# 1chizhang/OpenDCVC

Hardware: AMD Instinct MI355X
Metric: 1080p YUV420 encode+decode FPS (frames/s through encode AND decode, whole job) (higher is better)
Workload: dtype f16

## Files before the change

### opendcvc_amd/csrc/dcb_t128.hpp

```cpp
#pragma once

namespace t128 {

typedef float floatx16 __attribute__((ext_vector_type(16)));

constexpr int TW = 16, TH = 8, M = TW * TH;
constexpr int NW = 8, NTHR = NW * 64;
constexpr int PT = M / 32;
constexpr int PTW = PT / 2;
constexpr int PAD = 8;
constexpr int VC = 64, LDV = VC + PAD;
constexpr int HALO = (TH + 2) * (TW + 2);
constexpr int DW_SLAB = 64;
constexpr int LDS_S = DW_SLAB;

constexpr int PADF = 24;

struct G128 {
    static constexpr int TW = t128::TW, TH = t128::TH, NW = t128::NW, D = 8, DW_SLAB = t128::DW_SLAB, WPS = 2;
};
struct G32 {
    static constexpr int TW = 8, TH = 4, NW = 4, D = 24 , DW_SLAB = 128, WPS = 1;
};
template <class G>
struct Geo : G {
    static constexpr int M = G::TW * G::TH, NTHR = G::NW * 64;
    static constexpr int PTW = (M / 32) / (G::NW / 4);
    static constexpr int HALO = (G::TH + 2) * (G::TW + 2);
    static constexpr int LDS_S = G::DW_SLAB;
    static_assert(M % 32 == 0 && PTW >= 1 && G::NW % 4 == 0, "tile geometry");
};

template <int C>
struct Wcfg {
    static_assert(C % 64 == 0, "DepthConvBlock widths are padded to 64");
    static constexpr int NT = C / 32;
    static constexpr int NTW = (NT + 3) / 4;
    static constexpr bool RAG = NT % 4 != 0;
    static constexpr int KS = C / 16;
    static constexpr int NCH = 2 * C / VC;
    static constexpr int F4 = 4 * NTW;
    static constexpr int LDX = C + PAD;
    static constexpr int FRAGS = KS * NTW + NCH * KS + NCH * F4;
    static constexpr int STREAM = FRAGS + PADF;
};

template <int C, class G = G128, bool HEADIN = false>
struct Cfg : Wcfg<C> {
    using GE = Geo<G>;
    using WC = Wcfg<C>;
    using WC::NT; using WC::NTW; using WC::RAG; using WC::KS; using WC::NCH; using WC::F4; using WC::LDX; using WC::FRAGS; using WC::STREAM;
    static_assert(C % G::DW_SLAB == 0, "whole depthwise slabs");
    static constexpr int D = G::D;
    static_assert(D <= PADF, "stream padding");
    static constexpr size_t slab_elems = (size_t)(HEADIN && C / G::DW_SLAB > 2 ? C / G::DW_SLAB : 2) * GE::HALO * GE::LDS_S;
    static constexpr size_t v_elems = (size_t)2 * GE::M * LDV > slab_elems ? (size_t)2 * GE::M * LDV : slab_elems;
    static constexpr size_t TAB_BYTES = (size_t)9 * C * 2 + (size_t)C * 4 + (size_t)4 * C * 4;
    static constexpr int HROWS = (GE::HALO + 31) / 32 * 32;
    static constexpr size_t HEAD_BYTES = HEADIN ? (size_t)HROWS * LDX * sizeof(half_t) : 0;
    static constexpr size_t LDS = ((size_t)GE::M * LDX + v_elems) * sizeof(half_t) + TAB_BYTES + HEAD_BYTES;
    static_assert(LDS <= 160 * 1024, "LDS budget");
    static_assert(NCH % 2 == 0 && NCH >= 4, "the chunk loop is unrolled by two");
    static_assert((2 * C) % VC == 0, "whole FFN chunks");
    static constexpr int OFF_U0 = (KS * NTW) % D;
    static constexpr int OFF_S0 = (OFF_U0 + KS) % D;
    static constexpr int OFF_ODD = (OFF_S0 + KS) % D;
    static constexpr int OFF_EVEN = (OFF_ODD + F4 + KS) % D;
    static_assert((2 * (F4 + KS)) % D == 0, "the two-step loop body must turn the ring a whole number of times");
    static constexpr int OFF_LAST = OFF_ODD;
    static constexpr int OFF_FIN = (OFF_LAST + F4) % D;
};

__device__ __forceinline__ floatx16 mfma32(const half8& a, const half8& b, const floatx16& c)
{
    return __builtin_amdgcn_mfma_f32_32x32x16_f16(a, b, c, 0, 0, 0);
}


template <int C, class G = G128, bool HEADIN = false>
__global__ __launch_bounds__(Geo<G>::NTHR, G::WPS) void dcb_tail128_kernel(TailParams p)
{
    using TR = Traits<half_t>;
    using CF = Cfg<C, G, HEADIN>;
    using GE = Geo<G>;
    constexpr int TW = GE::TW, TH = GE::TH, M = GE::M, NTHR = GE::NTHR, PTW = GE::PTW, HALO = GE::HALO, DW_SLAB = GE::DW_SLAB,
                  LDS_S = GE::LDS_S;
    constexpr int NTW = CF::NTW, KS = CF::KS, NCH = CF::NCH, D = CF::D, LDX = CF::LDX, V = 8, GC = C / V;
    extern __shared__ __attribute__((aligned(32))) char smem[];
    half_t* bufX = reinterpret_cast<half_t*>(smem);
    half_t* bufV = bufX + M * LDX;
    half_t* tabW = bufV + CF::v_elems;
    float* tabBd = reinterpret_cast<float*>(tabW + 9 * C);
    float* tabB3 = tabBd + C;
    const int tid = threadIdx.x, lane = tid & 63;
    const int wave = __builtin_amdgcn_readfirstlane(tid >> 6);
    const int cqw = wave & 3, ph = wave >> 2;
    const int pl = lane & 31, hh = lane >> 5;
    const int tiles_x = (p.W + TW - 1) / TW;
    const int ty0 = (blockIdx.x / tiles_x) * TH, tx0 = (blockIdx.x % tiles_x) * TW;
    const half_t* a = reinterpret_cast<const half_t*>(p.a);
    const half_t* ident = reinterpret_cast<const half_t*>(p.ident);
    [[maybe_unused]] unsigned long long ts0 = 0, ts1 = 0, ts2 = 0, ts3 = 0, ts4 = 0, ts5 = 0, ts6 = 0;
    [[maybe_unused]] unsigned long long td[8] = {0, 0, 0, 0, 0, 0, 0, 0};
    STAMP(ts0);

    const __amdgpu_buffer_rsrc_t wrsrc = __builtin_amdgcn_make_buffer_rsrc(
        const_cast<char*>(reinterpret_cast<const char*>(p.wt)) + (size_t)cqw * CF::STREAM * 1024, 0, CF::STREAM * 1024, 0x00020000);
    const int wlane = lane * 16;
    int woff = 0;
    auto wload = [&]() __attribute__((always_inline)) {
        typedef unsigned u32x4 __attribute__((ext_vector_type(4)));
        const u32x4 v = __builtin_amdgcn_raw_buffer_load_b128(wrsrc, wlane, woff, 0);
        woff += 1024;
        return __builtin_bit_cast(half8, v);
    };
    half8 ring[D];

    constexpr int HW_ = TW + 2, GS = DW_SLAB / V, NLD = (HALO * GS + NTHR - 1) / NTHR;
    constexpr int nslab = C / DW_SLAB;
// ... 99 lines not shown
        }
#pragma unroll
        for (int i = 0; i < NTW; ++i) {
            const int chb = 32 * (cqw + 4 * i) + 4 * hh;
#pragma unroll
            for (int g = 0; g < 4; ++g) {
                const floatx4 bias = load_f4(p.hb1 + chb + 8 * g);
#pragma unroll
                for (int t = 0; t < HT; ++t) {
                    const int hp = 32 * t + pl;
                    const int y = ty0 - 1 + hp / HW_, x = tx0 - 1 + hp % HW_;
                    const bool inside = hp < HALO && y >= 0 && y < p.H && x >= 0 && x < p.W;
                    floatx4 v = {hacc[i][t][4 * g], hacc[i][t][4 * g + 1], hacc[i][t][4 * g + 2], hacc[i][t][4 * g + 3]};
                    v = v + bias;
#pragma unroll
                    for (int r = 0; r < 4; ++r) v[r] = inside ? TR::gate(v[r]) : 0.f;
                    const int ch = chb + 8 * g;
                    if (hp < HALO) lds_store_quad<half_t>(bufV + (ch / DW_SLAB) * (HALO * LDS_S), LDS_S, hp, ch % DW_SLAB, v);
                }
            }
        }
    }
    constexpr int NID = M * GC / NTHR;
    constexpr int G8 = C / 64, RPP = NTHR / 8;
    static_assert(M % RPP == 0 && NID == (M / RPP) * G8, "identity pass mapping");
    auto idmap = [&](int k, int& m, int& c) __attribute__((always_inline)) {
        c = ((tid & 7) + 8 * (k % G8)) * V;
        m = (tid >> 3) + RPP * (k / G8);
    };
    Vec16 idv[NID];
    const __amdgpu_buffer_rsrc_t irsrc = __builtin_amdgcn_make_buffer_rsrc(
        const_cast<half_t*>(ident), 0, (int)((long)p.H * p.W * p.ldi * 2), 0x00020000);
    auto ident_fetch = [&]() __attribute__((always_inline)) {
#pragma unroll
        for (int k = 0; k < NID; ++k) {
            int m, icg;
            idmap(k, m, icg);
            const int y = ty0 + m / TW, x = tx0 + m % TW;
            int off = (y < p.H && x < p.W) ? ((y * p.W + x) * (int)p.ldi + icg) * 2 : OOB;
#ifdef DCVC_DIAG
            if (p.ablate & 32) off = (tid & 255) * 16;
#endif
            idv[k] = __builtin_bit_cast(Vec16, __builtin_amdgcn_raw_buffer_load_b128(irsrc, off, 0, 0));
        }
    };

    const int prow = (ph * PTW) * 32 + pl;
    const half_t* xb = bufX + prow * LDX + 8 * hh;
    auto bfrag_x = [&](int t, int s) __attribute__((always_inline)) {
        return *reinterpret_cast<const half8*>(xb + t * 32 * LDX + s * 16);
    };

    floatx16 acc[NTW][PTW];
    half8 g2b[PTW];
    auto gemm2_slot = [&](int s, int q) __attribute__((always_inline)) {
        const int i = q / PTW, t = q % PTW, k = (s * NTW + i) % D;
        if (q == 0) {
#pragma unroll
            for (int tt = 0; tt < PTW; ++tt) g2b[tt] = bfrag_x(tt, s);
        }
        if (s == 0) {
            floatx16 zero;
#pragma unroll
            for (int r = 0; r < 16; ++r) zero[r] = 0.f;
            acc[i][t] = mfma32(ring[k], g2b[t], zero);
        } else {
            acc[i][t] = mfma32(ring[k], g2b[t], acc[i][t]);
        }
        if (t == PTW - 1) ring[k] = wload();
    };
    constexpr int G2Q = NTW * PTW;
    {
        static_assert(NTHR / GS == M / 2 && TH % 2 == 0, "one pixel pair per thread and slab");
        const int pp = tid / GS, py = 2 * (pp / TW), px = pp % TW;
#pragma unroll
        for (int slab = 0; slab < nslab; ++slab) {
            half_t* hb = bufV + (HEADIN ? slab : (slab & 1)) * (HALO * LDS_S);
            if constexpr (!HEADIN) {
#pragma unroll
                for (int k = 0; k < NLD; ++k) {
                    const int hp = tid / GS + k * (NTHR / GS);
                    if (hp < HALO) *reinterpret_cast<Vec16*>(hb + hp * LDS_S + dcs) = pre[slab][k];
                }
            }
            if (slab == (nslab >= 2 ? nslab - 2 : 0)) ident_fetch();
            if (slab == nslab - 1) {
#pragma unroll
                for (int k = 0; k < D; ++k) ring[k] = wload();
            }
            if (slab == 0) STAMP(td[0]);
            __syncthreads();
            if (slab < 4) STAMP(td[1 + slab]);
            taps_fetch(slab);
            const int c = slab * DW_SLAB + dcs;
            Vec16 tv[4][3];
#pragma unroll
            for (int r = 0; r < 4; ++r)
#pragma unroll
                for (int kx = 0; kx < 3; ++kx)
                    tv[r][kx] = *reinterpret_cast<const Vec16*>(hb + ((py + r) * HW_ + px + kx) * LDS_S + dcs);
            __builtin_amdgcn_sched_barrier(0);
#pragma unroll
            for (int e = 0; e < 2; ++e) {
                float sacc[V];
#pragma unroll
                for (int j = 0; j < V; ++j) sacc[j] = 0.f;
#pragma unroll
                for (int ky = 0; ky < 3; ++ky)
#pragma unroll
                    for (int kx = 0; kx < 3; ++kx) fma_vec16<half_t>(tv[e + ky][kx], wtap[ky * 3 + kx], sacc);
#pragma unroll
                for (int j = 0; j < 4; ++j) {
                    sacc[j] = sacc[j] + bd0[j];
                    sacc[4 + j] = sacc[4 + j] + bd1[j];
                }
                lds_store_vec<half_t>(bufX, LDX, (py + e) * TW + px, c, pack16<half_t>(sacc));
            }
        }
        __syncthreads();
    }
    STAMP(ts1);

    auto tile_of = [&](int i) __attribute__((always_inline)) { return cqw + 4 * i; };
    auto tile_exists = [&](int i) __attribute__((always_inline)) { return !CF::RAG || cqw + 4 * i < CF::NT; };
    constexpr bool EB_PRE = NTW <= 2;
    floatx4 ebias[EB_PRE ? NTW : 1][4];
    auto ebias_load = [&](const float* b) __attribute__((always_inline)) {
        if constexpr (EB_PRE) {
#pragma unroll
            for (int i = 0; i < NTW; ++i)
#pragma unroll
                for (int g = 0; g < 4; ++g) ebias[i][g] = load_f4(b + 32 * tile_of(i) + 4 * hh + 8 * g);
        }
    };
    auto ebias_get = [&](const float* b, int i, int g) __attribute__((always_inline)) {
        if constexpr (EB_PRE) return ebias[i][g];
        return load_f4(b + 32 * tile_of(i) + 4 * hh + 8 * g);
    };
    ebias_load(p.b2);

#pragma unroll
    for (int mm = 0; mm < KS * G2Q; ++mm) {
        gemm2_slot(mm / G2Q, mm % G2Q);
        __builtin_amdgcn_sched_barrier(0);
    }
    auto gemm_c = [&](auto next) __attribute__((always_inline)) {
        half8 bc[PTW], bn[PTW];
#pragma unroll
        for (int t = 0; t < PTW; ++t) bc[t] = bfrag_x(t, 0);
        floatx16 zero;
#pragma unroll
        for (int r = 0; r < 16; ++r) zero[r] = 0.f;
        __builtin_amdgcn_sched_barrier(0);
#pragma unroll
        for (int s = 0; s < KS; ++s) {
// ... 27 lines not shown
    }
    __syncthreads();
#pragma unroll
    for (int k = 0; k < NID; ++k) {
        int m, icg;
        idmap(k, m, icg);
        const half8 o = __builtin_bit_cast(half8, lds_load_vec<half_t>(bufX, LDX, m, icg)) + __builtin_bit_cast(half8, idv[k]);
        lds_store_vec<half_t>(bufX, LDX, m, icg, __builtin_bit_cast(Vec16, o));
    }
    __syncthreads();

    STAMP(ts3);
#pragma unroll
    for (int i = 0; i < NTW; ++i)
#pragma unroll
        for (int t = 0; t < PTW; ++t)
#pragma unroll
            for (int r = 0; r < 16; ++r) acc[i][t][r] = 0.f;
    floatx16 ua[PTW], ub[PTW];
    const float* b3w = tabB3 + 16 * cqw + 4 * hh;
    floatx16 biasv;
    auto bias_load = [&](int j) __attribute__((always_inline)) {
        j = j < NCH ? j : NCH - 1;
        const floatx4 l0 = load_f4(b3w + 64 * j), l1 = load_f4(b3w + 64 * j + 8);
        const floatx4 h0 = load_f4(b3w + 64 * j + 2 * C), h1 = load_f4(b3w + 64 * j + 2 * C + 8);
#pragma unroll
        for (int r = 0; r < 4; ++r) {
            biasv[r] = l0[r];
            biasv[4 + r] = l1[r];
            biasv[8 + r] = h0[r];
            biasv[12 + r] = h1[r];
        }
    };
    constexpr int NPIECE = 4 * PTW * 6;
    float ge[4], gr[4];
    floatx4 vq;
    auto gate_piece = [&](const floatx16 (&u)[PTW], half_t* vbuf, int i) __attribute__((always_inline)) {
        const int n = i / 6, phs = i % 6, t = n >> 2, g = (n >> 1) & 1, hf = n & 1;
        const float lo0 = u[t][4 * g + 2 * hf], lo1 = u[t][4 * g + 2 * hf + 1];
        const float hi0 = u[t][8 + 4 * g + 2 * hf], hi1 = u[t][8 + 4 * g + 2 * hf + 1];
        if (phs == 0) {
            ge[0] = __builtin_amdgcn_exp2f(lo0);
            ge[1] = __builtin_amdgcn_exp2f(lo1);
        } else if (phs == 1) {
            ge[2] = __builtin_amdgcn_exp2f(hi0);
            ge[3] = __builtin_amdgcn_exp2f(hi1);
        } else if (phs == 2) {
            gr[0] = __builtin_amdgcn_rcpf(1.0f + ge[0]);
// ... 1 lines not shown
        } else if (phs == 3) {
            gr[2] = __builtin_amdgcn_rcpf(1.0f + ge[2]);
            gr[3] = __builtin_amdgcn_rcpf(1.0f + ge[3]);
        } else if (phs == 4) {
            vq[2 * hf] = DCVC_FMAF(hi0, gr[2], lo0 * gr[0]);
        } else {
            vq[2 * hf + 1] = DCVC_FMAF(hi1, gr[3], lo1 * gr[1]);
            if (hf == 1) lds_store_quad<half_t>(vbuf, LDV, prow + 32 * t, 16 * cqw + 8 * g + 4 * hh, vq);
        }
    };
    auto wload_ffn = [&]() __attribute__((always_inline)) {
#ifdef DCVC_DIAG
        if (p.ablate & 256) {
            typedef unsigned u32x4 __attribute__((ext_vector_type(4)));
            return __builtin_bit_cast(half8, __builtin_amdgcn_raw_buffer_load_b128(wrsrc, wlane, 0, 0));
        }
#endif
        return wload();
    };
    auto step = [&](auto G4c, auto G3c, auto GATEc, auto OFFc, const floatx16 (&ug)[PTW], floatx16 (&un)[PTW], half_t* vcur,
                    const half_t* vprev, int jb) __attribute__((always_inline)) {
        constexpr bool G4 = decltype(G4c)::value, G3 = decltype(G3c)::value, GATE = decltype(GATEc)::value;
        constexpr int OFF = decltype(OFFc)::value;
        constexpr int N4 = G4 ? 4 : 0, NS = N4 + (G3 ? KS : 0);
        constexpr int TM = N4 * NTW * PTW + (G3 ? KS * PTW : 0);
        constexpr int PPS = GATE ? (NPIECE + TM - 1) / TM : 0;
        auto load_b1 = [&](int idx, int t) __attribute__((always_inline)) {
#ifdef DCVC_DIAG
            if (p.ablate & 512) idx = idx < N4 ? 0 : N4;
#endif
            if (idx < N4) return *reinterpret_cast<const half8*>(vprev + (prow + 32 * t) * LDV + 8 * hh + idx * 16);
            return bfrag_x(t, idx - N4);
        };
        half8 bc[PTW], bn[PTW];
#pragma unroll
        for (int t = 0; t < PTW; ++t) bc[t] = load_b1(0, t);
        __builtin_amdgcn_sched_barrier(0);
        int m = 0;
#pragma unroll
        for (int idx = 0; idx < NS; ++idx) {
            const int nm = idx < N4 ? NTW * PTW : PTW;
#pragma unroll
            for (int q = 0; q < NTW * PTW; ++q) {
                if (q < nm) {
                    if (idx + 1 < NS && q < PTW) bn[q] = load_b1(idx + 1, q);
                    const int t = q % PTW;
                    if (idx < N4) {
// ... 638 lines not shown
```

### opendcvc_amd/csrc/dcvc_nn.hip

```cpp
#include <algorithm>
#include <cstdio>
#include <cstdlib>
#include <functional>
#include <memory>
#include <mutex>
#include <type_traits>
#include <unordered_map>
#include <vector>

#include "common.hpp"
#include "gemm_core.hpp"

namespace {

using dcvc::round_up;

template <int MT>
struct Tile {
    static constexpr int M = 16 * MT;
    static constexpr int TW = MT >= 8 ? 16 : 8;
    static constexpr int TH = M / TW;
};

#ifndef DCVC_PF_SMALL
// ... 841 lines not shown
{
    std::vector<float> v(n);
    for (int i = 0; i < n; ++i) v[i] = get(i);
    return dst.upload(v.data(), v.size() * sizeof(float));
}

template <typename T>
int upload_T(DevBuf& dst, int n, const std::function<float(int)>& get)
{
    std::vector<T> v(n);
    for (int i = 0; i < n; ++i) v[i] = (T)get(i);
    return dst.upload(v.data(), v.size() * sizeof(T));
}


}

struct dcvc_dcb {
    int dtype, cin, c, cin_p, c_p, shortcut, adapt;
    DevBuf wa, ba, w1, b1, wd, bd, w2, b2, w3, b3, w4, b4;
    DevBuf wa_t128;
    DevBuf w1_t128;
    DevBuf wt128;
};

struct dcvc_conv {
    int dtype, cin, cout, cin_p, n_p, cs_p, kh, kw, stride, pad, epi;
    DevBuf w, b;
    DevBuf w_t128;
    DevBuf w_c128[2];
    DevBuf w_s2;
};

namespace {

template <typename T, int MT>
size_t head_lds(int kstage, int c, bool adapt)
{
    const int kx = kstage > c ? kstage : c;
    return (size_t)Tile<MT>::M * ((kx + Traits<T>::kPad) + (adapt ? c + Traits<T>::kPad : 0)) * sizeof(T);
}
template <typename T, int MT, int NTW, int NW>
size_t tail_lds(int c)
{
    return TailLds<T, MT, TailCfg<MT, NTW, NW>::NTV, NW>::bytes(c);
}

template <typename T, int MT, int NTW, int NW, bool RAG = false, bool HEADIN = false>
int launch_tail(const TailParams& tp, int grid, int C, hipStream_t st)
{
    const size_t lds = TailLds<T, MT, TailCfg<MT, NTW, NW>::NTV, NW>::bytes(C, HEADIN);
    int rc = set_lds(dcb_tail_kernel<T, MT, NTW, NW, RAG, HEADIN>, lds);
// ... 4 lines not shown

template <typename K>
int set_lds(K kernel, size_t bytes)
{
    if (bytes > 160 * 1024) {
        dcvc::set_error("kernel needs %zu bytes of LDS (> 160 KiB)", bytes);
        return dcvc::E_ARG;
    }
    if (bytes > 64 * 1024) {
        static std::mutex mu;
        static std::unordered_map<const void*, size_t> granted;
        const void* key = reinterpret_cast<const void*>(kernel);
        std::lock_guard<std::mutex> lk(mu);
        size_t& have = granted[key];
        if (have < bytes) {
            DCVC_HIP(hipFuncSetAttribute(key, hipFuncAttributeMaxDynamicSharedMemorySize, (int)bytes));
            have = bytes;
        }
    }
    return 0;
}


template <int C>
int pack_t128(DevBuf& dst, const std::function<float(int, int)>& W2, const std::function<float(int, int)>& W3,
              const std::function<float(int, int)>& W4)
{
    using CF = t128::Wcfg<C>;
    std::vector<half_t> buf((size_t)4 * CF::STREAM * 512, (half_t)0.f);
    for (int wave = 0; wave < 4; ++wave) {
        size_t f = 0;
        auto put = [&](const std::function<float(int, int)>& get, const std::function<int(int)>& row, int s) {
            half_t* o = &buf[((size_t)wave * CF::STREAM + f) * 512];
            for (int l = 0; l < 64; ++l)
                for (int j = 0; j < 8; ++j) o[l * 8 + j] = (half_t)get(row(l & 31), 16 * s + 8 * (l >> 5) + j);
            ++f;
        };
        auto g3 = [&](int j) {
            for (int s = 0; s < CF::KS; ++s)
                put(W3, [&](int r) { return (r < 16 ? 0 : 2 * C - 16) + 64 * j + 16 * wave + r; }, s);
        };
        auto g4 = [&](int j) {
            for (int s4 = 0; s4 < 4; ++s4)
                for (int i = 0; i < CF::NTW; ++i) put(W4, [&](int r) { return 32 * (wave + 4 * i) + r; }, 4 * j + s4);
        };
        for (int s = 0; s < CF::KS; ++s)
            for (int i = 0; i < CF::NTW; ++i) put(W2, [&](int r) { return 32 * (wave + 4 * i) + r; }, s);
        g3(0);
        for (int j = 0; j < CF::NCH; ++j) {
            if (j >= 1) g4(j - 1);
            if (j + 1 < CF::NCH) g3(j + 1);
        }
        g4(CF::NCH - 1);
        if (f != (size_t)CF::FRAGS) {
            dcvc::set_error("pack_t128: %zu fragments packed, %d expected", f, CF::FRAGS);
            return dcvc::E_ARG;
        }
    }
    return dst.upload(buf.data(), buf.size() * sizeof(half_t));
}

inline bool t128_width_ok(int c_p) { return c_p == 128 || c_p == 256 || c_p == 320 || c_p == 384 || c_p == 512; }

template <int C>
int pack_t128_square(DevBuf& dst, const std::function<float(int, int)>& W)
{
    using CF = t128::Wcfg<C>;
    constexpr int LEN = CF::KS * CF::NTW + t128::PADF;
    std::vector<half_t> buf((size_t)4 * LEN * 512, (half_t)0.f);
    for (int cq = 0; cq < 4; ++cq) {
        size_t f = 0;
        for (int s = 0; s < CF::KS; ++s)
            for (int i = 0; i < CF::NTW; ++i, ++f) {
                half_t* o = &buf[((size_t)cq * LEN + f) * 512];
                for (int l = 0; l < 64; ++l)
                    for (int j = 0; j < 8; ++j) o[l * 8 + j] = (half_t)W(32 * (cq + 4 * i) + (l & 31), 16 * s + 8 * (l >> 5) + j);
            }
    }
    return dst.upload(buf.data(), buf.size() * sizeof(half_t));
}

template <int C>
int pack_t128_rect(DevBuf& dst, int Kp, const std::function<float(int, int)>& W)
{
    using CF = t128::Wcfg<C>;
    const int ks = Kp / 16, LEN = ks * CF::NTW + t128::PADF;
    std::vector<half_t> buf((size_t)4 * LEN * 512, (half_t)0.f);
    for (int cq = 0; cq < 4; ++cq) {
        size_t f = 0;
        for (int s = 0; s < ks; ++s)
            for (int i = 0; i < CF::NTW; ++i, ++f) {
                half_t* o = &buf[((size_t)cq * LEN + f) * 512];
                for (int l = 0; l < 64; ++l)
                    for (int j = 0; j < 8; ++j) o[l * 8 + j] = (half_t)W(32 * (cq + 4 * i) + (l & 31), 16 * s + 8 * (l >> 5) + j);
            }
    }
    return dst.upload(buf.data(), buf.size() * sizeof(half_t));
}

// ... 15 lines not shown
                    }
        }
    return dst.upload(buf.data(), buf.size() * sizeof(half_t));
}

template <typename F>
int visit_t128_width(int c_p, F&& f)
{
    switch (c_p) {
    case 128: return f(std::integral_constant<int, 128>());
    case 256: return f(std::integral_constant<int, 256>());
    case 320: return f(std::integral_constant<int, 320>());
    case 384: return f(std::integral_constant<int, 384>());
    case 512: return f(std::integral_constant<int, 512>());
    default: dcvc::set_error("no fragment-stream form for width %d", c_p); return dcvc::E_ARG;
    }
}

inline int pack_t128_square_any(int c_p, DevBuf& dst, const std::function<float(int, int)>& W)
{
    return visit_t128_width(c_p, [&](auto w) { return pack_t128_square<decltype(w)::value>(dst, W); });
}

struct Switches {
    bool t128, t32, h128, c128;
#ifdef DCVC_DIAG
    int mt, conv_mt, ablate;
    bool stamps;
#endif
};

static const Switches& switches()
{
    static const Switches sw = [] {
        auto on = [](const char* name) { const char* v = getenv(name); return !(v && atoi(v) == 0); };
        auto num = [](const char* name) { const char* v = getenv(name); return v ? atoi(v) : 0; };
        Switches s{};
        s.t128 = on("DCVC_T128");
        s.t32 = on("DCVC_T32");
        s.h128 = on("DCVC_H128");
        s.c128 = on("DCVC_C128");
#ifdef DCVC_DIAG
        s.mt = num("DCVC_MT");
        s.conv_mt = num("DCVC_CONV_MT");
        s.ablate = num("DCVC_ABLATE");
        s.stamps = getenv("DCVC_STAMPS") != nullptr;
#endif
        (void)num;
        return s;
    }();
    return sw;
}

template <typename K, typename P>
int launch_kernel(K kernel, dim3 grid, int threads, size_t lds, hipStream_t st, const P& p)
{
    int rc = set_lds(kernel, lds);
    if (rc) return rc;
    hipLaunchKernelGGL(kernel, grid, dim3(threads), lds, st, p);
    return 0;
}

#ifdef DCVC_DIAG
static int stamp_medians(unsigned long long* d, int grid, int per, const char* const* names, const char* tag, int& calls,
// ... 12 lines not shown
        for (int b = 0; b < grid; ++b) v[b] = hs[(size_t)b * per + k];
        std::sort(v.begin(), v.end());
        fprintf(stderr, " %s=%llu", names[k], v[grid / 2]);
    }
    return 0;
}
#endif

template <int C, class G = t128::G128, bool HEADIN = false>
int launch_tail128(const TailParams& tp, int H, int W, hipStream_t st)
{
    const int grid = ((H + G::TH - 1) / G::TH) * ((W + G::TW - 1) / G::TW);
    const size_t lds = t128::Cfg<C, G, HEADIN>::LDS;
#ifdef DCVC_DIAG
    if (switches().stamps) {
        TailParams q = tp;
        DCVC_HIP(hipMalloc(&q.stamps, (size_t)grid * 16 * sizeof(unsigned long long)));
        int rc = launch_kernel(t128::dcb_tail128_kernel<C, G, HEADIN>, dim3(grid), t128::Geo<G>::NTHR, lds, st, q);
        if (rc) return rc;
        const char* names[16] = {"loads+dw", "gemm2", "o_pass", "u0", "ffn", "r+store", nullptr, nullptr, "dw:issue+stage0",
                                 "barrier0", "slab0", "slab1", "slab2", "slab3", "fused", nullptr};
        for (int k = C / G::DW_SLAB; k < 4; ++k) names[10 + k] = nullptr;
        char tag[64];
        snprintf(tag, sizeof tag, "t128 stamps C=%d tile=%d grid=%d", C, t128::Geo<G>::M, grid);
        static int calls = 0;
        std::vector<unsigned long long> hs;
        bool printed = false;
        rc = stamp_medians(q.stamps, grid, 16, names, tag, calls, st, hs, printed);
        if (rc || !printed) return rc;
        std::vector<unsigned long long> du(grid);
        for (int b = 0; b < grid; ++b) du[b] = hs[(size_t)b * 16 + 7] - hs[(size_t)b * 16 + 6];
        std::sort(du.begin(), du.end());
        fprintf(stderr, " | wg total min/med/max %llu %llu %llu\n", du[0], du[grid / 2], du[grid - 1]);
        return 0;
    }
#endif
    return launch_kernel(t128::dcb_tail128_kernel<C, G, HEADIN>, dim3(grid), t128::Geo<G>::NTHR, lds, st, tp);
}

struct ChainArgs {
    int head_done = 0, a_slot = 0;
    int separate_head = 0;
    const dcvc_dcb* next = nullptr;
    const dcvc_conv* conv = nullptr;
    const float* conv_q = nullptr;
    void* conv_out = nullptr;
    int64_t ldco = 0;
};

static int pick_mt_f16(int H, int W)
{
#ifdef DCVC_DIAG
    if (switches().mt == 2 || switches().mt == 4) return switches().mt;
#endif
    return (long)H * W >= 12000 ? 4 : 2;
}

constexpr bool has_tail128(bool f16, int mt, int ntw, bool headin)
{
    return f16 && (mt == 4 ? !headin && (ntw == 4 || ntw == 5 || ntw == 6)
                           : headin ? (ntw == 2 || ntw == 4) : (ntw == 4 || ntw == 6 || ntw == 8));
}
constexpr bool has_head128(bool f16, int mt, int ntw)
{
    return f16 && (mt == 4 ? (ntw == 4 || ntw == 5 || ntw == 6) : (ntw == 4 || ntw == 6 || ntw == 8));
}
constexpr bool has_tail_headin(bool f16, int mt, int ntw) { return f16 && mt == 2 && (ntw <= 4 || ntw == 6); }

struct TailForm {
    int ntw, nw;
    bool rag;
};
constexpr TailForm tail_form(bool f16, int ntw)
{
    return !f16 ? TailForm{ntw, 4, false} : ntw == 5 ? TailForm{3, 8, true}
                                          : ntw >= 6 && ntw % 2 == 0 ? TailForm{ntw / 2, 8, false} : TailForm{ntw, 4, false};
}

struct DcbPlan {
    enum class Head { none, head128, head } head = Head::none;
    bool head_adapt = false;
    bool head_t32 = false;
    enum class Tail { tail128, tail } tail = Tail::tail;
    bool headin = false;
    int mt = 2, ntw = 1;
    TailForm form{1, 4, false};
    const void* nwt = nullptr;
};

static DcbPlan plan_dcb(const dcvc_dcb* h, const SrcPair& src, int H, int W, const ChainArgs& ch)
{
    const Switches& sw = switches();
    const bool f16 = h->dtype == DCVC_F16;
    DcbPlan pl;
    pl.mt = f16 ? pick_mt_f16(H, W) : 2;
    pl.ntw = h->c_p / 64;
    const int mt = pl.mt, ntw = pl.ntw;
    pl.nwt = ch.next ? ch.next->w1_t128.p : ch.conv ? ch.conv->w_t128.p : nullptr;
    const bool t128 = sw.t128 && h->wt128.p != nullptr && (pl.nwt != nullptr || (!ch.next && !ch.conv));
    const bool own_head = !ch.head_done && !ch.separate_head && !h->adapt && src.c1 == 0;

    if (has_tail128(f16, mt, ntw, true) && t128 && sw.t32 && h->w1_t128.p != nullptr && own_head) {
        pl.tail = DcbPlan::Tail::tail128;
        pl.headin = true;
    } else if (has_tail128(f16, mt, ntw, false) && t128 && (mt == 4 || sw.t32)) {
        pl.tail = DcbPlan::Tail::tail128;
    } else {
        pl.tail = DcbPlan::Tail::tail;
        pl.headin = has_tail_headin(f16, mt, ntw) && own_head;
        pl.form = tail_form(f16, ntw);
    }

    const int kin = src.c0 + src.c1;
    if (ch.head_done || pl.headin) {
        pl.head = DcbPlan::Head::none;
    } else if (sw.t128 && sw.h128 && has_head128(f16, mt, ntw) && (mt == 4 || pl.tail == DcbPlan::Tail::tail128) &&
               h->w1_t128.p != nullptr &&
               (h->adapt ? (h->wa_t128.p != nullptr && src.c0 % 64 == 0 && src.c1 % 64 == 0 && kin == h->cin_p)
                         : (src.c1 == 0 && src.c0 == ntw * 64))) {
        pl.head = DcbPlan::Head::head128;
        pl.head_adapt = h->adapt;
    } else {
        pl.head = DcbPlan::Head::head;
        pl.head_adapt = h->adapt;
        const int kstage = src.c1 > 0 ? std::max(src.c0, src.c1) : kin;
        pl.head_t32 = h->adapt && mt == 4 && head_lds<half_t, 4>(kstage, h->c_p, true) > 80 * 1024;
    }
    return pl;
}
// ... 39 lines not shown
    tp.ident = h->adapt ? (const void*)id_buf : src.x0;
    tp.ldi = h->adapt ? C : src.ld0;
    tp.H = H;
    tp.W = W;
    tp.C = C;
    tp.c_log = h->c;
    tp.wd = h->wd.p;
    tp.bd = (const float*)h->bd.p;
    tp.w2 = h->w2.p;
    tp.b2 = (const float*)h->b2.p;
    tp.w3 = h->w3.p;
    tp.b3 = (const float*)h->b3.p;
    tp.w4 = h->w4.p;
    tp.b4 = (const float*)h->b4.p;
    tp.shortcut = h->shortcut;
    tp.q = quant;
    tp.out = out;
    tp.ldo = ldo;
    tp.hx = src.x0;
    tp.ldhx = src.ld0;
    tp.hw1 = h->w1.p;
    tp.hb1 = (const float*)h->b1.p;
    tp.hwt = h->w1_t128.p;
    tp.wt = h->wt128.p;
    tp.nwt = pl.nwt;
    if (ch.next) {
        tp.nw1 = ch.next->w1.p;
        tp.nb1 = (const float*)ch.next->b1.p;
        tp.na_out = a_next;
        tp.nlda = C;
    } else if (ch.conv) {
        tp.nw1 = ch.conv->w.p;
        tp.nb1 = (const float*)ch.conv->b.p;
        tp.na_out = ch.conv_out;
        tp.nlda = ch.ldco;
        tp.nplain = 1;
        tp.nq = ch.conv_q;
        tp.n_log = ch.conv->cout;
    }
#ifdef DCVC_DIAG
    tp.ablate = switches().ablate;
#endif

    if (ev) DCVC_HIP(hipEventRecord(ev[0], st));
    int rc = 0;
    if (pl.head == DcbPlan::Head::head128) {
        if constexpr (has_head128(f16, MT, NTW)) {
// ... 3 lines not shown
                               : launch_kernel(t128::dcb_head128_kernel<NTW * 64, false, G>, g128, t128::Geo<G>::NTHR, lds, st, hp);
        } else {
            rc = not_built("dcb_head128_kernel", pl);
        }
    } else if (pl.head == DcbPlan::Head::head) {
        const int kstage = pl.head_adapt && hp.split ? std::max(src.c0, src.c1) : src.c0 + src.c1;
        if (!pl.head_adapt) {
            rc = launch_kernel(dcb_head_kernel<T, MT, NTW, false>, dim3(grid), NTHREADS, head_lds<T, MT>(kstage, C, false), st, hp);
        } else if (pl.head_t32) {
            const int grid2 = ((H + Tile<2>::TH - 1) / Tile<2>::TH) * ((W + Tile<2>::TW - 1) / Tile<2>::TW);
            rc = launch_kernel(dcb_head_kernel<T, 2, NTW, true>, dim3(grid2), NTHREADS, head_lds<T, 2>(kstage, C, true), st, hp);
        } else {
            rc = launch_kernel(dcb_head_kernel<T, MT, NTW, true>, dim3(grid), NTHREADS, head_lds<T, MT>(kstage, C, true), st, hp);
        }
    }
    if (rc) return rc;
    DCVC_LAUNCH_CHECK();
    if (ev) DCVC_HIP(hipEventRecord(ev[1], st));

    if (pl.tail == DcbPlan::Tail::tail128) {
        if (pl.headin) {
            if constexpr (has_tail128(f16, MT, NTW, true)) rc = launch_tail128<NTW * 64, G, true>(tp, H, W, st);
            else rc = not_built("dcb_tail128_kernel<..., HEADIN>", pl);
        } else {
            if constexpr (has_tail128(f16, MT, NTW, false)) rc = launch_tail128<NTW * 64, G>(tp, H, W, st);
            else rc = not_built("dcb_tail128_kernel", pl);
        }
        if (rc) return rc;
        DCVC_LAUNCH_CHECK();
    } else {
        constexpr TailForm F = tail_form(f16, NTW);
#ifdef DCVC_DIAG
        if (switches().stamps) DCVC_HIP(hipMalloc(&tp.stamps, (size_t)grid * 8 * sizeof(unsigned long long)));
#endif
        if (pl.headin) {
            if constexpr (has_tail_headin(f16, MT, NTW)) rc = launch_tail<T, MT, F.ntw, F.nw, F.rag, true>(tp, grid, C, st);
            else rc = not_built("dcb_tail_kernel<..., HEADIN>", pl);
        } else {
            rc = launch_tail<T, MT, F.ntw, F.nw, F.rag>(tp, grid, C, st);
        }
        if (rc) return rc;
        DCVC_LAUNCH_CHECK();
#ifdef DCVC_DIAG
        if (tp.stamps) {
            const char* names[8] = {"dw", "gemm2", "o_pass", "gemm3", "ffn_epi", "gemm4", "final", "total"};
            char tag[64];
// ... 201 lines not shown
    const float ka = dtype == DCVC_F16 ? Traits<half_t>::kAct : 1.0f;
    rc |= pack_any(dtype, h->w1, Cp, Cp, [&](int n, int k) { return (n < C && k < C) ? ka * w1[(size_t)n * C + k] : 0.f; });
    rc |= upload_f32(h->b1, Cp, [&](int n) { return n < C ? ka * b1[n] : 0.f; });
    auto dwget = [&](int i) { const int t = i / Cp, ch = i % Cp; return ch < C ? wd[(size_t)ch * 9 + t] / ka : 0.f; };
    rc |= dtype == DCVC_F16 ? upload_T<half_t>(h->wd, 9 * Cp, dwget) : upload_T<float>(h->wd, 9 * Cp, dwget);
    rc |= upload_f32(h->bd, Cp, [&](int n) { return n < C ? bd[n] : 0.f; });
    rc |= pack_any(dtype, h->w2, Cp, Cp, [&](int n, int k) { return (n < C && k < C) ? w2[(size_t)n * C + k] : 0.f; });
    rc |= upload_f32(h->b2, Cp, [&](int n) { return n < C ? b2[n] : 0.f; });
    auto u_row = [&](int n) { const int half = n / (2 * Cp), cc = n % (2 * Cp); return cc < 2 * C ? half * 2 * C + cc : -1; };
    rc |= pack_any(dtype, h->w3, 4 * Cp, Cp, [&](int n, int k) { const int rr = u_row(n); return (rr >= 0 && k < C) ? ka * w3[(size_t)rr * C + k] : 0.f; });
    rc |= upload_f32(h->b3, 4 * Cp, [&](int n) { const int rr = u_row(n); return rr >= 0 ? ka * b3[rr] : 0.f; });
    rc |= pack_any(dtype, h->w4, Cp, 2 * Cp, [&](int n, int k) { return (n < C && k < 2 * C) ? w4[(size_t)n * 2 * C + k] / ka : 0.f; });
    rc |= upload_f32(h->b4, Cp, [&](int n) { return n < C ? b4[n] : 0.f; });
    if (rc == 0 && dtype == DCVC_F16 && t128_width_ok(Cp)) {
        auto W2 = [&](int n, int k) { return (n < C && k < C) ? w2[(size_t)n * C + k] : 0.f; };
        auto W3 = [&](int n, int k) { const int rr = u_row(n); return (rr >= 0 && k < C) ? ka * w3[(size_t)rr * C + k] : 0.f; };
        auto W4 = [&](int n, int k) { return (n < C && k < 2 * C) ? w4[(size_t)n * 2 * C + k] / ka : 0.f; };
        if (h->adapt && Kp % 64 == 0) {
            auto WA = [&](int n, int k) { return (n < C && k < cin) ? adaptor_w[(size_t)n * cin + k] : 0.f; };
            rc |= visit_t128_width(Cp, [&](auto w) { return pack_t128_rect<decltype(w)::value>(h->wa_t128, Kp, WA); });
        }
        rc |= pack_t128_square_any(Cp, h->w1_t128, [&](int n, int k) { return (n < C && k < C) ? ka * w1[(size_t)n * C + k] : 0.f; });
        rc |= visit_t128_width(Cp, [&](auto w) { return pack_t128<decltype(w)::value>(h->wt128, W2, W3, W4); });
    }
    if (rc) return rc < 0 ? rc : dcvc::E_MEM;
    *out = h.release();
    return 0;
}

void dcvc_dcb_destroy(dcvc_dcb* h) { delete h; }

size_t dcvc_dcb_scratch_bytes(const dcvc_dcb* h, int H, int W)
{
    if (!h) return 0;
    return (size_t)H * W * h->c_p * dcvc::elem_size(h->dtype) * 3;
}

int dcvc_dcb_forward(const dcvc_dcb* h, const void* x0, int64_t ld0, int c0, const void* x1, int64_t ld1, int c1,
                     int H, int W, const float* quant, void* out, int64_t ldo, void* scratch, void* stream)
{
    return dcvc_dcb_forward_chained(h, x0, ld0, c0, x1, ld1, c1, H, W, quant, out, ldo, scratch, stream, 0, 0, nullptr);
}

int dcvc_dcb_forward_chained(const dcvc_dcb* h, const void* x0, int64_t ld0, int c0, const void* x1, int64_t ld1, int c1,
                             int H, int W, const float* quant, void* out, int64_t ldo, void* scratch, void* stream,
                             int head_done, int a_slot, const dcvc_dcb* next)
// ... 132 lines not shown
    h->stride = stride;
    h->pad = pad;
    h->epi = epilogue;
    const int Kp = h->cin_p = round_up(cin, 32);
    const int taps = kh * kw;
    int Np;
    std::function<int(int)> to_log;
    if (epilogue == DCVC_EPI_SHUFFLE2) {
        const int cs = cout / 4, csp = h->cs_p = round_up(cs, 32);
        Np = 4 * csp;
        to_log = [=](int n) { const int s = n / csp, cc = n % csp; return cc < cs ? cc * 4 + s : -1; };
    } else {
        h->cs_p = 0;
        Np = round_up(cout, 32);
        to_log = [=](int n) { return n < cout ? n : -1; };
    }
    h->n_p = Np;
    int rc = pack_any(dtype, h->w, Np, taps * Kp, [&](int n, int k) {
        const int nl = to_log(n), t = k / Kp, ci = k % Kp;
        return (nl >= 0 && ci < cin) ? w[((size_t)nl * cin + ci) * taps + t] : 0.f;
    });
    rc |= upload_f32(h->b, Np, [&](int n) { const int nl = to_log(n); return nl >= 0 ? b[nl] : 0.f; });
    if (rc == 0 && dtype == DCVC_F16 && taps == 1 && epilogue != DCVC_EPI_SHUFFLE2 && Np == Kp && Np == round_up(cout, 64) && t128_width_ok(Np))
        rc |= pack_t128_square_any(Np, h->w_t128, [&](int n, int k) { return (n < cout && k < cin) ? w[(size_t)n * cin + k] : 0.f; });
    if (rc == 0 && dtype == DCVC_F16 && kh == 3 && kw == 3 && stride == 1 && pad == 1 && Kp % 64 == 0 && Kp <= 256 && Np % 256 == 0 &&
        (epilogue == DCVC_EPI_BIAS || (epilogue == DCVC_EPI_SHUFFLE2 && h->cs_p % 256 == 0))) {
        auto WC = [&](int n, int t, int ci) {
            const int nl = to_log(n);
            return (nl >= 0 && ci < cin) ? w[((size_t)nl * cin + ci) * taps + t] : 0.f;
        };
        rc |= pack_t128_conv(h->w_c128[0], 1, 9, 4, Np, Kp, WC);
        rc |= pack_t128_conv(h->w_c128[1], 2, 9, 8, Np, Kp, WC);
    }
    if (rc == 0 && dtype == DCVC_F16 && stride == 2 && ((kh == 2 && kw == 2 && pad == 0) || (kh == 3 && kw == 3 && pad == 1)) &&
        Kp % 128 == 0 && Kp <= 384 && (Np == 128 || Np == 256) && epilogue == DCVC_EPI_BIAS)
        rc |= pack_t128_conv(h->w_s2, Np / 128, taps, 8 * (Np / 128), Np, Kp, [&](int n, int t, int ci) {
            const int nl = to_log(n);
            return (nl >= 0 && ci < cin) ? w[((size_t)nl * cin + ci) * taps + t] : 0.f;
        });
    if (rc) return rc < 0 ? rc : dcvc::E_MEM;
    *out = h.release();
    return 0;
}

void dcvc_conv_destroy(dcvc_conv* h) { delete h; }

int dcvc_conv_forward(const dcvc_conv* h, const void* x0, int64_t ld0, int c0, const void* x1, int64_t ld1, int c1,
// ... 46 lines not shown
```

Baseline: 437.1.

## Add eight-wave channel-eighths variant of the 32-pixel DepthConvBlock tail kernel

Introduces a G32W8 geometry in which eight waves each own one eighth of the output channels (NQ=8), instead of four waves splitting quarters. Weight streams are repacked per eighth, and the identity, depthwise and FFN chunk mappings are generalised to the new wave count. The plan selects it by default for 512-wide blocks (ntw==8) on the 32-pixel tile path, with an environment override. The goal is more waves per block and shorter per-wave weight streams on the widest layers, at the cost of extra packed weight copies and possibly lower per-wave reuse and occupancy.

```diff
diff --git a/opendcvc_amd/csrc/dcb_t128.hpp b/opendcvc_amd/csrc/dcb_t128.hpp
--- a/opendcvc_amd/csrc/dcb_t128.hpp
+++ b/opendcvc_amd/csrc/dcb_t128.hpp
@@ -17,51 +17,58 @@
 constexpr int PADF = 24;
 
 struct G128 {
-    static constexpr int TW = t128::TW, TH = t128::TH, NW = t128::NW, D = 8, DW_SLAB = t128::DW_SLAB, WPS = 2;
+    static constexpr int TW = t128::TW, TH = t128::TH, NW = t128::NW, NQ = 4, D = 8, DW_SLAB = t128::DW_SLAB, WPS = 2;
 };
 struct G32 {
-    static constexpr int TW = 8, TH = 4, NW = 4, D = 24 , DW_SLAB = 128, WPS = 1;
+    static constexpr int TW = 8, TH = 4, NW = 4, NQ = 4, D = 24 , DW_SLAB = 128, WPS = 1;
+};
+struct G32W8 {
+    static constexpr int TW = 8, TH = 4, NW = 8, NQ = 8, D = 16 , DW_SLAB = 128, WPS = 1;
 };
 template <class G>
 struct Geo : G {
     static constexpr int M = G::TW * G::TH, NTHR = G::NW * 64;
-    static constexpr int PTW = (M / 32) / (G::NW / 4);
+    static constexpr int PTW = (M / 32) / (G::NW / G::NQ);
     static constexpr int HALO = (G::TH + 2) * (G::TW + 2);
     static constexpr int LDS_S = G::DW_SLAB;
-    static_assert(M % 32 == 0 && PTW >= 1 && G::NW % 4 == 0, "tile geometry");
+    static constexpr int VC = 16 * G::NQ, LDV = VC + PAD;
+    static_assert(M % 32 == 0 && PTW >= 1 && G::NW % G::NQ == 0, "tile geometry");
 };
 
-template <int C>
+template <int C, int NQ = 4>
 struct Wcfg {
     static_assert(C % 64 == 0, "DepthConvBlock widths are padded to 64");
+    static_assert(NQ == 4 || NQ == 8, "channel quarters or eighths");
     static constexpr int NT = C / 32;
-    static constexpr int NTW = (NT + 3) / 4;
-    static constexpr bool RAG = NT % 4 != 0;
+    static constexpr int NTW = (NT + NQ - 1) / NQ;
+    static constexpr bool RAG = NT % NQ != 0;
     static constexpr int KS = C / 16;
+    static constexpr int VC = 16 * NQ;
     static constexpr int NCH = 2 * C / VC;
-    static constexpr int F4 = 4 * NTW;
+    static constexpr int N4 = VC / 16;
+    static constexpr int F4 = N4 * NTW;
     static constexpr int LDX = C + PAD;
     static constexpr int FRAGS = KS * NTW + NCH * KS + NCH * F4;
     static constexpr int STREAM = FRAGS + PADF;
 };
 
 template <int C, class G = G128, bool HEADIN = false>
-struct Cfg : Wcfg<C> {
+struct Cfg : Wcfg<C, G::NQ> {
     using GE = Geo<G>;
-    using WC = Wcfg<C>;
-    using WC::NT; using WC::NTW; using WC::RAG; using WC::KS; using WC::NCH; using WC::F4; using WC::LDX; using WC::FRAGS; using WC::STREAM;
+    using WC = Wcfg<C, G::NQ>;
+    using WC::NT; using WC::NTW; using WC::RAG; using WC::KS; using WC::NCH; using WC::N4; using WC::F4; using WC::LDX; using WC::FRAGS; using WC::STREAM;
     static_assert(C % G::DW_SLAB == 0, "whole depthwise slabs");
     static constexpr int D = G::D;
     static_assert(D <= PADF, "stream padding");
     static constexpr size_t slab_elems = (size_t)(HEADIN && C / G::DW_SLAB > 2 ? C / G::DW_SLAB : 2) * GE::HALO * GE::LDS_S;
-    static constexpr size_t v_elems = (size_t)2 * GE::M * LDV > slab_elems ? (size_t)2 * GE::M * LDV : slab_elems;
+    static constexpr size_t v_elems = (size_t)2 * GE::M * GE::LDV > slab_elems ? (size_t)2 * GE::M * GE::LDV : slab_elems;
     static constexpr size_t TAB_BYTES = (size_t)9 * C * 2 + (size_t)C * 4 + (size_t)4 * C * 4;
     static constexpr int HROWS = (GE::HALO + 31) / 32 * 32;
     static constexpr size_t HEAD_BYTES = HEADIN ? (size_t)HROWS * LDX * sizeof(half_t) : 0;
     static constexpr size_t LDS = ((size_t)GE::M * LDX + v_elems) * sizeof(half_t) + TAB_BYTES + HEAD_BYTES;
     static_assert(LDS <= 160 * 1024, "LDS budget");
     static_assert(NCH % 2 == 0 && NCH >= 4, "the chunk loop is unrolled by two");
-    static_assert((2 * C) % VC == 0, "whole FFN chunks");
+    static_assert((2 * C) % WC::VC == 0, "whole FFN chunks");
     static constexpr int OFF_U0 = (KS * NTW) % D;
     static constexpr int OFF_S0 = (OFF_U0 + KS) % D;
     static constexpr int OFF_ODD = (OFF_S0 + KS) % D;
@@ -84,7 +91,7 @@
     using CF = Cfg<C, G, HEADIN>;
     using GE = Geo<G>;
     constexpr int TW = GE::TW, TH = GE::TH, M = GE::M, NTHR = GE::NTHR, PTW = GE::PTW, HALO = GE::HALO, DW_SLAB = GE::DW_SLAB,
-                  LDS_S = GE::LDS_S;
+                  LDS_S = GE::LDS_S, VC = GE::VC, LDV = GE::LDV, NQ = G::NQ;
     constexpr int NTW = CF::NTW, KS = CF::KS, NCH = CF::NCH, D = CF::D, LDX = CF::LDX, V = 8, GC = C / V;
     extern __shared__ __attribute__((aligned(32))) char smem[];
     half_t* bufX = reinterpret_cast<half_t*>(smem);
@@ -94,7 +101,7 @@
     float* tabB3 = tabBd + C;
     const int tid = threadIdx.x, lane = tid & 63;
     const int wave = __builtin_amdgcn_readfirstlane(tid >> 6);
-    const int cqw = wave & 3, ph = wave >> 2;
+    const int cqw = wave % NQ, ph = wave / NQ;
     const int pl = lane & 31, hh = lane >> 5;
     const int tiles_x = (p.W + TW - 1) / TW;
     const int ty0 = (blockIdx.x / tiles_x) * TH, tx0 = (blockIdx.x % tiles_x) * TW;
@@ -240,11 +247,12 @@
         }
     }
     constexpr int NID = M * GC / NTHR;
-    constexpr int G8 = C / 64, RPP = NTHR / 8;
-    static_assert(M % RPP == 0 && NID == (M / RPP) * G8, "identity pass mapping");
+    constexpr int TPP = NTHR / 8 > M ? NTHR / M : 8;
+    constexpr int G8 = C / (8 * TPP), RPP = NTHR / TPP;
+    static_assert(M % RPP == 0 && C % (8 * TPP) == 0 && NID == (M / RPP) * G8, "identity pass mapping");
     auto idmap = [&](int k, int& m, int& c) __attribute__((always_inline)) {
-        c = ((tid & 7) + 8 * (k % G8)) * V;
-        m = (tid >> 3) + RPP * (k / G8);
+        c = ((tid % TPP) + TPP * (k % G8)) * V;
+        m = (tid / TPP) + RPP * (k / G8);
     };
     Vec16 idv[NID];
     const __amdgpu_buffer_rsrc_t irsrc = __builtin_amdgcn_make_buffer_rsrc(
@@ -289,8 +297,9 @@
     };
     constexpr int G2Q = NTW * PTW;
     {
-        static_assert(NTHR / GS == M / 2 && TH % 2 == 0, "one pixel pair per thread and slab");
-        const int pp = tid / GS, py = 2 * (pp / TW), px = pp % TW;
+        constexpr int PPT = M * GS / NTHR;
+        static_assert((PPT == 1 || PPT == 2) && NTHR / GS * PPT == M && TH % PPT == 0, "one pixel (pair) per thread and slab");
+        const int pp = tid / GS, py = PPT * (pp / TW), px = pp % TW;
 #pragma unroll
         for (int slab = 0; slab < nslab; ++slab) {
             half_t* hb = bufV + (HEADIN ? slab : (slab & 1)) * (HALO * LDS_S);
@@ -311,15 +320,15 @@
             if (slab < 4) STAMP(td[1 + slab]);
             taps_fetch(slab);
             const int c = slab * DW_SLAB + dcs;
-            Vec16 tv[4][3];
-#pragma unroll
-            for (int r = 0; r < 4; ++r)
+            Vec16 tv[PPT + 2][3];
+#pragma unroll
+            for (int r = 0; r < PPT + 2; ++r)
 #pragma unroll
                 for (int kx = 0; kx < 3; ++kx)
                     tv[r][kx] = *reinterpret_cast<const Vec16*>(hb + ((py + r) * HW_ + px + kx) * LDS_S + dcs);
             __builtin_amdgcn_sched_barrier(0);
 #pragma unroll
-            for (int e = 0; e < 2; ++e) {
+            for (int e = 0; e < PPT; ++e) {
                 float sacc[V];
 #pragma unroll
                 for (int j = 0; j < V; ++j) sacc[j] = 0.f;
@@ -339,8 +348,8 @@
     }
     STAMP(ts1);
 
-    auto tile_of = [&](int i) __attribute__((always_inline)) { return cqw + 4 * i; };
-    auto tile_exists = [&](int i) __attribute__((always_inline)) { return !CF::RAG || cqw + 4 * i < CF::NT; };
+    auto tile_of = [&](int i) __attribute__((always_inline)) { return cqw + NQ * i; };
+    auto tile_exists = [&](int i) __attribute__((always_inline)) { return !CF::RAG || cqw + NQ * i < CF::NT; };
     constexpr bool EB_PRE = NTW <= 2;
     floatx4 ebias[EB_PRE ? NTW : 1][4];
     auto ebias_load = [&](const float* b) __attribute__((always_inline)) {
@@ -348,7 +357,8 @@
 #pragma unroll
             for (int i = 0; i < NTW; ++i)
 #pragma unroll
-                for (int g = 0; g < 4; ++g) ebias[i][g] = load_f4(b + 32 * tile_of(i) + 4 * hh + 8 * g);
+                for (int g = 0; g < 4; ++g)
+                    ebias[i][g] = load_f4(b + 32 * (tile_exists(i) ? tile_of(i) : cqw) + 4 * hh + 8 * g);
         }
     };
     auto ebias_get = [&](const float* b, int i, int g) __attribute__((always_inline)) {
@@ -422,8 +432,8 @@
     floatx16 biasv;
     auto bias_load = [&](int j) __attribute__((always_inline)) {
         j = j < NCH ? j : NCH - 1;
-        const floatx4 l0 = load_f4(b3w + 64 * j), l1 = load_f4(b3w + 64 * j + 8);
-        const floatx4 h0 = load_f4(b3w + 64 * j + 2 * C), h1 = load_f4(b3w + 64 * j + 2 * C + 8);
+        const floatx4 l0 = load_f4(b3w + VC * j), l1 = load_f4(b3w + VC * j + 8);
+        const floatx4 h0 = load_f4(b3w + VC * j + 2 * C), h1 = load_f4(b3w + VC * j + 2 * C + 8);
 #pragma unroll
         for (int r = 0; r < 4; ++r) {
             biasv[r] = l0[r];
@@ -471,7 +481,7 @@
                     const half_t* vprev, int jb) __attribute__((always_inline)) {
         constexpr bool G4 = decltype(G4c)::value, G3 = decltype(G3c)::value, GATE = decltype(GATEc)::value;
         constexpr int OFF = decltype(OFFc)::value;
-        constexpr int N4 = G4 ? 4 : 0, NS = N4 + (G3 ? KS : 0);
+        constexpr int N4 = G4 ? CF::N4 : 0, NS = N4 + (G3 ? KS : 0);
         constexpr int TM = N4 * NTW * PTW + (G3 ? KS * PTW : 0);
         constexpr int PPS = GATE ? (NPIECE + TM - 1) / TM : 0;
         auto load_b1 = [&](int idx, int t) __attribute__((always_inline)) {
diff --git a/opendcvc_amd/csrc/dcvc_nn.hip b/opendcvc_amd/csrc/dcvc_nn.hip
--- a/opendcvc_amd/csrc/dcvc_nn.hip
+++ b/opendcvc_amd/csrc/dcvc_nn.hip
@@ -887,12 +887,14 @@
     DevBuf wa_t128;
     DevBuf w1_t128;
     DevBuf wt128;
+    DevBuf w1_t128e, wt128e;
 };
 
 struct dcvc_conv {
     int dtype, cin, cout, cin_p, n_p, cs_p, kh, kw, stride, pad, epi;
     DevBuf w, b;
     DevBuf w_t128;
+    DevBuf w_t128e;
     DevBuf w_c128[2];
     DevBuf w_s2;
 };
@@ -943,13 +945,13 @@
 }
 
 
-template <int C>
+template <int C, int NQ = 4>
 int pack_t128(DevBuf& dst, const std::function<float(int, int)>& W2, const std::function<float(int, int)>& W3,
               const std::function<float(int, int)>& W4)
 {
-    using CF = t128::Wcfg<C>;
-    std::vector<half_t> buf((size_t)4 * CF::STREAM * 512, (half_t)0.f);
-    for (int wave = 0; wave < 4; ++wave) {
+    using CF = t128::Wcfg<C, NQ>;
+    std::vector<half_t> buf((size_t)NQ * CF::STREAM * 512, (half_t)0.f);
+    for (int wave = 0; wave < NQ; ++wave) {
         size_t f = 0;
         auto put = [&](const std::function<float(int, int)>& get, const std::function<int(int)>& row, int s) {
             half_t* o = &buf[((size_t)wave * CF::STREAM + f) * 512];
@@ -959,14 +961,14 @@
         };
         auto g3 = [&](int j) {
             for (int s = 0; s < CF::KS; ++s)
-                put(W3, [&](int r) { return (r < 16 ? 0 : 2 * C - 16) + 64 * j + 16 * wave + r; }, s);
+                put(W3, [&](int r) { return (r < 16 ? 0 : 2 * C - 16) + CF::VC * j + 16 * wave + r; }, s);
         };
         auto g4 = [&](int j) {
-            for (int s4 = 0; s4 < 4; ++s4)
-                for (int i = 0; i < CF::NTW; ++i) put(W4, [&](int r) { return 32 * (wave + 4 * i) + r; }, 4 * j + s4);
+            for (int s4 = 0; s4 < CF::N4; ++s4)
+                for (int i = 0; i < CF::NTW; ++i) put(W4, [&](int r) { return 32 * (wave + NQ * i) + r; }, CF::N4 * j + s4);
         };
         for (int s = 0; s < CF::KS; ++s)
-            for (int i = 0; i < CF::NTW; ++i) put(W2, [&](int r) { return 32 * (wave + 4 * i) + r; }, s);
+            for (int i = 0; i < CF::NTW; ++i) put(W2, [&](int r) { return 32 * (wave + NQ * i) + r; }, s);
         g3(0);
         for (int j = 0; j < CF::NCH; ++j) {
             if (j >= 1) g4(j - 1);
@@ -982,20 +984,21 @@
 }
 
 inline bool t128_width_ok(int c_p) { return c_p == 128 || c_p == 256 || c_p == 320 || c_p == 384 || c_p == 512; }
-
-template <int C>
+inline bool t128_eighths_ok(int c_p) { return c_p == 256 || c_p == 384 || c_p == 512; }
+
+template <int C, int NQ = 4>
 int pack_t128_square(DevBuf& dst, const std::function<float(int, int)>& W)
 {
-    using CF = t128::Wcfg<C>;
+    using CF = t128::Wcfg<C, NQ>;
     constexpr int LEN = CF::KS * CF::NTW + t128::PADF;
-    std::vector<half_t> buf((size_t)4 * LEN * 512, (half_t)0.f);
-    for (int cq = 0; cq < 4; ++cq) {
+    std::vector<half_t> buf((size_t)NQ * LEN * 512, (half_t)0.f);
+    for (int cq = 0; cq < NQ; ++cq) {
         size_t f = 0;
         for (int s = 0; s < CF::KS; ++s)
             for (int i = 0; i < CF::NTW; ++i, ++f) {
                 half_t* o = &buf[((size_t)cq * LEN + f) * 512];
                 for (int l = 0; l < 64; ++l)
-                    for (int j = 0; j < 8; ++j) o[l * 8 + j] = (half_t)W(32 * (cq + 4 * i) + (l & 31), 16 * s + 8 * (l >> 5) + j);
+                    for (int j = 0; j < 8; ++j) o[l * 8 + j] = (half_t)W(32 * (cq + NQ * i) + (l & 31), 16 * s + 8 * (l >> 5) + j);
             }
     }
     return dst.upload(buf.data(), buf.size() * sizeof(half_t));
@@ -1057,8 +1060,25 @@
     return visit_t128_width(c_p, [&](auto w) { return pack_t128_square<decltype(w)::value>(dst, W); });
 }
 
+template <typename F>
+int visit_t128_eighths(int c_p, F&& f)
+{
+    switch (c_p) {
+    case 256: return f(std::integral_constant<int, 256>());
+    case 384: return f(std::integral_constant<int, 384>());
+    case 512: return f(std::integral_constant<int, 512>());
+    default: dcvc::set_error("no eight-stream form for width %d", c_p); return dcvc::E_ARG;
+    }
+}
+
+inline int pack_t128_square_eighths(int c_p, DevBuf& dst, const std::function<float(int, int)>& W)
+{
+    return visit_t128_eighths(c_p, [&](auto w) { return pack_t128_square<decltype(w)::value, 8>(dst, W); });
+}
+
 struct Switches {
     bool t128, t32, h128, c128;
+    int t32w8;
 #ifdef DCVC_DIAG
     int mt, conv_mt, ablate;
     bool stamps;
@@ -1075,6 +1095,7 @@
         s.t32 = on("DCVC_T32");
         s.h128 = on("DCVC_H128");
         s.c128 = on("DCVC_C128");
+        s.t32w8 = getenv("DCVC_T32W8") ? (atoi(getenv("DCVC_T32W8")) != 0) : -1;
 #ifdef DCVC_DIAG
         s.mt = num("DCVC_MT");
         s.conv_mt = num("DCVC_CONV_MT");
@@ -1133,7 +1154,7 @@
                                  "barrier0", "slab0", "slab1", "slab2", "slab3", "fused", nullptr};
         for (int k = C / G::DW_SLAB; k < 4; ++k) names[10 + k] = nullptr;
         char tag[64];
-        snprintf(tag, sizeof tag, "t128 stamps C=%d tile=%d grid=%d", C, t128::Geo<G>::M, grid);
+        snprintf(tag, sizeof tag, "t128 stamps C=%d tile=%d waves=%d grid=%d", C, t128::Geo<G>::M, G::NW, grid);
         static int calls = 0;
         std::vector<unsigned long long> hs;
         bool printed = false;
@@ -1172,6 +1193,7 @@
     return f16 && (mt == 4 ? !headin && (ntw == 4 || ntw == 5 || ntw == 6)
                            : headin ? (ntw == 2 || ntw == 4) : (ntw == 4 || ntw == 6 || ntw == 8));
 }
+constexpr bool has_tail32w8(bool f16, int mt, int ntw) { return f16 && mt == 2 && (ntw == 4 || ntw == 6 || ntw == 8); }
 constexpr bool has_head128(bool f16, int mt, int ntw)
 {
     return f16 && (mt == 4 ? (ntw == 4 || ntw == 5 || ntw == 6) : (ntw == 4 || ntw == 6 || ntw == 8));
@@ -1194,6 +1216,7 @@
     bool head_t32 = false;
     enum class Tail { tail128, tail } tail = Tail::tail;
     bool headin = false;
+    bool w8 = false;
     int mt = 2, ntw = 1;
     TailForm form{1, 4, false};
     const void* nwt = nullptr;
@@ -1216,6 +1239,13 @@
         pl.headin = true;
     } else if (has_tail128(f16, mt, ntw, false) && t128 && (mt == 4 || sw.t32)) {
         pl.tail = DcbPlan::Tail::tail128;
+        const void* nwt8 = ch.next ? ch.next->w1_t128e.p : ch.conv ? ch.conv->w_t128e.p : nullptr;
+        const bool w8_default = ntw == 8;
+        if (mt == 2 && has_tail32w8(f16, mt, ntw) && h->wt128e.p != nullptr && (nwt8 != nullptr || (!ch.next && !ch.conv)) &&
+            (sw.t32w8 < 0 ? w8_default : sw.t32w8 != 0)) {
+            pl.w8 = true;
+            pl.nwt = nwt8;
+        }
     } else {
         pl.tail = DcbPlan::Tail::tail;
         pl.headin = has_tail_headin(f16, mt, ntw) && own_head;
@@ -1301,7 +1331,7 @@
     tp.hw1 = h->w1.p;
     tp.hb1 = (const float*)h->b1.p;
     tp.hwt = h->w1_t128.p;
-    tp.wt = h->wt128.p;
+    tp.wt = pl.w8 ? h->wt128e.p : h->wt128.p;
     tp.nwt = pl.nwt;
     if (ch.next) {
         tp.nw1 = ch.next->w1.p;
@@ -1351,6 +1381,9 @@
         if (pl.headin) {
             if constexpr (has_tail128(f16, MT, NTW, true)) rc = launch_tail128<NTW * 64, G, true>(tp, H, W, st);
             else rc = not_built("dcb_tail128_kernel<..., HEADIN>", pl);
+        } else if (pl.w8) {
+            if constexpr (has_tail32w8(f16, MT, NTW)) rc = launch_tail128<NTW * 64, t128::G32W8>(tp, H, W, st);
+            else rc = not_built("dcb_tail128_kernel<..., G32W8>", pl);
         } else {
             if constexpr (has_tail128(f16, MT, NTW, false)) rc = launch_tail128<NTW * 64, G>(tp, H, W, st);
             else rc = not_built("dcb_tail128_kernel", pl);
@@ -1598,6 +1631,10 @@
         }
         rc |= pack_t128_square_any(Cp, h->w1_t128, [&](int n, int k) { return (n < C && k < C) ? ka * w1[(size_t)n * C + k] : 0.f; });
         rc |= visit_t128_width(Cp, [&](auto w) { return pack_t128<decltype(w)::value>(h->wt128, W2, W3, W4); });
+        if (t128_eighths_ok(Cp)) {
+            rc |= pack_t128_square_eighths(Cp, h->w1_t128e, [&](int n, int k) { return (n < C && k < C) ? ka * w1[(size_t)n * C + k] : 0.f; });
+            rc |= visit_t128_eighths(Cp, [&](auto w) { return pack_t128<decltype(w)::value, 8>(h->wt128e, W2, W3, W4); });
+        }
     }
     if (rc) return rc < 0 ? rc : dcvc::E_MEM;
     *out = h.release();
@@ -1776,7 +1813,11 @@
     });
     rc |= upload_f32(h->b, Np, [&](int n) { const int nl = to_log(n); return nl >= 0 ? b[nl] : 0.f; });
     if (rc == 0 && dtype == DCVC_F16 && taps == 1 && epilogue != DCVC_EPI_SHUFFLE2 && Np == Kp && Np == round_up(cout, 64) && t128_width_ok(Np))
+    {
         rc |= pack_t128_square_any(Np, h->w_t128, [&](int n, int k) { return (n < cout && k < cin) ? w[(size_t)n * cin + k] : 0.f; });
+        if (t128_eighths_ok(Np))
+            rc |= pack_t128_square_eighths(Np, h->w_t128e, [&](int n, int k) { return (n < cout && k < cin) ? w[(size_t)n * cin + k] : 0.f; });
+    }
     if (rc == 0 && dtype == DCVC_F16 && kh == 3 && kw == 3 && stride == 1 && pad == 1 && Kp % 64 == 0 && Kp <= 256 && Np % 256 == 0 &&
         (epilogue == DCVC_EPI_BIAS || (epilogue == DCVC_EPI_SHUFFLE2 && h->cs_p % 256 == 0))) {
         auto WC = [&](int n, int t, int ci) {
```

New measurement: 433.1, median of 2. About the same (-0.9%).
